# rgcgithub/regenie

Measured on AMD Instinct MI355X. Metric: Step-1 SNPs x samples x phenos / sec, higher is better.
Workload: dtype fp4 (exact integer Gram) + i8 (exact fixed-point digit planes of the fp64 operands: G~X / G~Y, many-row predictions) + f64 (solves, level 1); 1 GPU; BASELINE configs[1]: synthetic PLINK bed 50000 samples x 100000 SNPs (100000 per GPU), 1 QT pheno, bsize 1000, 22 chromosomes, 5-fold CV, 5x5 ridge grid; `value` is the HBM-resident figure (packed genotypes generated on the device, timed region = level 0 + level 1 + LOCO rows); the complete run from files on disk is `end_to_end_from_files`; samples=50000, snps=100000, phenos=1, bsize=1000, blocks=109, parallelism=blocks sharded x1, all-gather of W, level-1 Gram tiles / ridge systems shared x1

## Files before the change

include/rg_step1.h:

```cpp
#ifndef RG_STEP1_H
#define RG_STEP1_H

#include <stdint.h>

#ifdef __cplusplus
extern "C" {
#endif

typedef struct rg_ctx rg_ctx;

#define RG_OK 0
#define RG_ERR_ARG (-1)
#define RG_ERR_HIP (-2)
#define RG_ERR_LOW_VARIANCE (-3)
#define RG_ERR_NOT_SPD (-4)
#define RG_ERR_STATE (-5)

#define RG_MEM_HOST 0
#define RG_MEM_DEVICE 1

typedef struct rg_problem {
  int64_t n_samples;
  int64_t n_file;
  int32_t n_pheno;
// ... 74 lines not shown
typedef struct rg_bt_options {
  int32_t niter_max_ridge;
  int32_t niter_max_line_search_ridge;
  int32_t niter_max_line_search;
  int32_t family;
  double l1_ridge_tol;
  double tol;
  double* beta_out;
  double* fold_cumsum_out;
} rg_bt_options;
int rg_l1_bt(rg_ctx* ctx, int32_t n_ridge_l1, const double* tau, const double* yraw,
             const double* offset, const rg_bt_options* opt, int32_t nchr,
             const int32_t* cols_per_chr, double* cumsum_out, int32_t* converged_out,
             int32_t* best_out, double* pred_out);

typedef struct rg_cox_options {
  int32_t niter_max;
  int32_t niter_max_line_search;
  int32_t niter_max_ridge;
  int32_t niter_max_line_search_ridge;
  double numtol_cox;
  double l1_ridge_tol;
  const double* tau;
} rg_cox_options;
int rg_l1_cox(rg_ctx* ctx, int32_t pheno, int32_t n_ridge_l1, const double* time, const double* event, const double* offset,
              const rg_cox_options* opt, int32_t nchr, const int32_t* cols_per_chr, double* tau_out, double* deviance_out,
              int32_t* converged_out, int32_t* best_out, double* pred_out);

typedef struct rg_timing {
  double ms_prep, ms_xy, ms_gram, ms_assemble, ms_chol, ms_solve, ms_pred, ms_l1_gram, ms_l1_chol,
      ms_l1_pred;
  int64_t n_gram_launches, n_chol_launches;
  double ms_wgram;
  double ms_irls_solve;
  double ms_irls_stream;
  int64_t n_wgram;
  int64_t n_irls_rounds;
  int64_t wgram_positions;
  int64_t n_wgram_approx_rounds;
  int64_t n_irls_passes;
} rg_timing;
int rg_enable_timing(rg_ctx* ctx, int on);
int rg_get_timing(rg_ctx* ctx, rg_timing* out);

int rg_k_gram_i8(void* stream, const uint8_t* A, int64_t lda, int a_miss, const uint8_t* B,
                 int64_t ldb, int b_miss, int32_t m, int32_t n, int64_t k_bytes, int32_t* C,
                 int64_t ldc);
int rg_k_gram_fp4(void* stream, const uint8_t* A4, int64_t lda, const uint8_t* B4, int64_t ldb,
                  int32_t m, int32_t n, int64_t k_bytes, int32_t* C, int64_t ldc);
int rg_k_chol_solve(void* stream, double* mats, int64_t mat_stride, int32_t batch, int32_t n_pad,
                    int32_t rhs_pad, int32_t nrhs ,
                    double* dinv_ws ,
                    int32_t* info );
int rg_k_dgemm_nt(void* stream, const double* A, int64_t lda, const double* B, int64_t ldb,
                  int32_t m, int32_t n, int64_t k, double* C, int64_t ldc);

int rg_k_xy_i8(void* stream, const uint8_t* pk, int64_t pk_ld, int64_t pk_blk_stride, int32_t nblk, int32_t n128,
               const int32_t* bs, const int32_t* nmiss, int32_t nseg, const int64_t* fold_len, const double* V, int64_t Np,
               int32_t Cv, int32_t route, int32_t* S32, int64_t s32_elems, double* part, int64_t part_elems,
               int32_t* nchunk_out);
int rg_k_wgram(void* stream, const double* W, int64_t Np, int32_t L, int32_t P, int32_t p, const double* wv, int32_t nchain,
               int32_t nseg, const int64_t* fold_len, const int32_t* slot_chain, int32_t nslot, int32_t excl_own, int32_t fmt,
               double* out, int32_t* nslice_out);

int rg_k_mfma_peak(int kind, int iters, double* tera_ops_out);

#ifdef __cplusplus
}
#endif
#endif
```

regenie_amd/csrc/chol_p128.h:

```cpp
#pragma once
#include "chol_common.h"

#ifndef RG_HOST_EMU
#define C128_LDS_ADDR(p) ((uint32_t)(uintptr_t)(__attribute__((address_space(3))) uint8_t*)(p))
#define C128_STAGE_SYNC() asm volatile("s_waitcnt vmcnt(0) lgkmcnt(0)\n\ts_barrier" ::: "memory")
#define c128_glds16 glds16
#define C128_RFL(x) __builtin_amdgcn_readfirstlane(x)
#define C128_LDS_BARRIER() asm volatile("s_waitcnt lgkmcnt(0)\n\ts_barrier" ::: "memory")
#define C128_LAUNDER(x) asm volatile("" : "+v"(x))
#define C128_STAGE_SYNC_ACC(acc)                                                                                                        \
  asm volatile("s_waitcnt vmcnt(0) lgkmcnt(0)\n\ts_barrier"                                                                            \
               : "+v"(acc[0][0]), "+v"(acc[0][1]), "+v"(acc[1][0]), "+v"(acc[1][1]), "+v"(acc[2][0]), "+v"(acc[2][1]), "+v"(acc[3][0]), \
                 "+v"(acc[3][1]), "+v"(acc[4][0]), "+v"(acc[4][1]), "+v"(acc[5][0]), "+v"(acc[5][1]), "+v"(acc[6][0]), "+v"(acc[6][1]), \
                 "+v"(acc[7][0]), "+v"(acc[7][1])                                                                                       \
               :                                                                                                                        \
               : "memory")
#define C128_STAGE_SYNC_ACCD(acc)                                                                                                       \
  asm volatile("s_waitcnt vmcnt(0) lgkmcnt(0)\n\ts_barrier"                                                                            \
               : "+v"(acc[0][0]), "+v"(acc[0][1]), "+v"(acc[1][0]), "+v"(acc[1][1]), "+v"(acc[2][0]), "+v"(acc[2][1]), "+v"(acc[3][0]), \
                 "+v"(acc[3][1]), "+v"(acc[4][1]), "+v"(acc[5][1]), "+v"(acc[6][1]), "+v"(acc[7][1])                                   \
               :                                                                                                                        \
               : "memory")
#else
#define C128_LAUNDER(x) ((void)0)
#define C128_LDS_BARRIER() __syncthreads()
#define C128_STAGE_SYNC_ACC(acc) C128_STAGE_SYNC()
#define C128_STAGE_SYNC_ACCD(acc) C128_STAGE_SYNC()
#endif

#define C128_UNIT 16384
#define C128_NBUF 4
#define C128_DIST 3
#ifndef RG_HOST_EMU
template <int N>
__device__ __forceinline__ void c128_wait_upto(int n) {
  if (N > 0 && n >= N) { asm volatile("s_waitcnt vmcnt(%0)" ::"n"(4 * N) : "memory"); return; }
  if (N > 0) c128_wait_upto<(N > 0 ? N - 1 : 0)>(n);
  else asm volatile("s_waitcnt vmcnt(0)" ::: "memory");
}
#define C128_UNIT_SYNC(later)                                          \
  do {                                                                 \
    c128_wait_upto<C128_DIST - 1>(later);                              \
    asm volatile("s_waitcnt lgkmcnt(0)\n\ts_barrier" ::: "memory");    \
  } while (0)
#else
#define C128_UNIT_SYNC(later) __syncthreads()
#endif
#define C128_STAGE 32768
#define C128_LDS (2 * C128_STAGE + 4096)

struct C128Args {
  double* mats; int64_t mat_stride; int n64;
  double* linv;
  double* dinv;
  int32_t* info;
  int j, Tp, batch, R, nplain;
  int flags;
  unsigned long long* dbg;
  FormSrc fs;
};
#ifndef RG_HOST_EMU
#define C128_T(k)                                                                        \
  do {                                                                                   \
    if (a.dbg && threadIdx.x == 0) {                                                     \
      const unsigned long long t_ = __builtin_amdgcn_s_memrealtime();                    \
      tl[k] += t_ - t_prev;                                                              \
      t_prev = t_;                                                                       \
    }                                                                                    \
  } while (0)
#define C128_TFLUSH()                                                                    \
  do {                                                                                   \
    if (a.dbg && threadIdx.x == 0)                                                       \
      for (int k_ = 1; k_ < 16; ++k_)                                                    \
        if (tl[k_]) atomicAdd(&a.dbg[k_], tl[k_]);                                       \
  } while (0)
#define C128_T0() (a.dbg ? __builtin_amdgcn_s_memrealtime() : 0ull)
#else
#define C128_T(k) ((void)0)
#define C128_TFLUSH() ((void)0)
#define C128_T0() 0ull
#endif

__device__ __forceinline__ bool c128_factor64(double (&s)[CT][CT + 2], double (&dv)[CT], unsigned long long* dbg = nullptr) {
#ifndef RG_HOST_EMU
#define C128_FT(k) do { if (dbg && threadIdx.x == 0) { const unsigned long long t_ = __builtin_amdgcn_s_memrealtime(); dbg[k] += t_ - tf; tf = t_; } } while (0)
  unsigned long long tf = dbg ? __builtin_amdgcn_s_memrealtime() : 0ull;
#else
#define C128_FT(k) ((void)0)
#endif
  const int tid = threadIdx.x;
  const int lane = tid & 63, wave = tid >> 6;
  const int li = lane & 15, lq = lane >> 4;
  auto inv_diag = [&](int o, int r, int c) -> double {
    return (c < r) ? s[o + c][o + r] : ((c == r) ? dv[o + r] : 0.0);
  };
  bool bad = false;
  for (int sb = 0; sb < 4; ++sb) {
    const int o = sb * 16;
    const int nb = 3 - sb;
    if (tid < 16) {
      double a[16], rdv[16];
#pragma unroll
      for (int c = 0; c < 16; ++c) a[c] = s[o + tid][o + c];
#pragma unroll
      for (int c = 0; c < 16; ++c) {
        const double p0 = bcast_lane(a[c], c);
        const bool ok = p0 > 0.0;
        bad |= !ok;
        const double piv = ok ? p0 : 1.0;
        double r0 = __builtin_amdgcn_rsq(piv);
        r0 = r0 * fma(-0.5 * piv * r0, r0, 1.5);
        r0 = r0 * fma(-0.5 * piv * r0, r0, 1.5);
        double d = piv * r0;
        d = fma(0.5 * r0, fma(-d, d, piv), d);
        const double rd = fma(r0, fma(-d, r0, 1.0), r0);
        rdv[c] = rd;
        a[c] = tid == c ? d : a[c] * rd;
#pragma unroll
        for (int c2 = c + 1; c2 < 16; ++c2) a[c2] = fma(-a[c], bcast_lane(a[c], c2), a[c2]);
      }
#pragma unroll
      for (int c = 0; c < 16; ++c)
        if (c <= tid) s[o + tid][o + c] = a[c];
      double v[16];
#pragma unroll
      for (int r = 0; r < 16; ++r) v[r] = (r == tid) ? 1.0 : 0.0;
#pragma unroll
      for (int j = 0; j < 16; ++j) {
        v[j] *= rdv[j];
#pragma unroll
        for (int r = j + 1; r < 16; ++r) v[r] = fma(-bcast_lane(a[j], r), v[j], v[r]);
      }
      dv[o + tid] = v[tid];
#pragma unroll
      for (int r = 0; r < 16; ++r)
        if (r > tid) s[o + tid][o + r] = v[r];
    }
    C128_FT(11);
    C128_LDS_BARRIER();
    C128_FT(14);
    if (wave < nb) {
      const int rb = o + 16 + 16 * wave;
      v4d acc = (v4d){0, 0, 0, 0};
#pragma unroll
      for (int st = 0; st < 4; ++st)
        acc = __builtin_amdgcn_mfma_f64_16x16x4f64(s[rb + li][o + 4 * lq + st], inv_diag(o, li, 4 * lq + st), acc, 0, 0, 0);
#pragma unroll
      for (int r = 0; r < 4; ++r) s[rb + lq + 4 * r][o + li] = acc[r];
    }
    C128_LDS_BARRIER();
    {
      const int nblk2 = nb * (nb + 1) / 2;
      for (int idx = wave; idx < nblk2; idx += 4) {
        int bi = 0, rem = idx;
        while (rem > bi) { rem -= bi + 1; ++bi; }
        const int bj = rem;
        const int ri = o + 16 + 16 * bi, rj = o + 16 + 16 * bj;
        v4d acc = (v4d){0, 0, 0, 0};
#pragma unroll
        for (int st = 0; st < 4; ++st)
          acc = __builtin_amdgcn_mfma_f64_16x16x4f64(s[ri + li][o + 4 * lq + st], s[rj + li][o + 4 * lq + st], acc, 0, 0, 0);
#pragma unroll
        for (int r = 0; r < 4; ++r)
          if (bi != bj || li <= lq + 4 * r) s[ri + lq + 4 * r][rj + li] -= acc[r];
      }
    }
    C128_LDS_BARRIER();
    C128_FT(12);
  }
  C128_FT(12);
  for (int dist = 1; dist < 4; ++dist) {
    const int j = wave, ib = wave + dist;
    if (ib < 4) {
      v4d m1 = (v4d){0, 0, 0, 0};
      for (int kb = j; kb < ib; ++kb) {
#pragma unroll
        for (int st = 0; st < 4; ++st) {
          const int kk = 4 * lq + st;
          const double bval = (kb == j) ? inv_diag(16 * j, kk, li) : s[16 * j + li][16 * kb + kk];
          m1 = __builtin_amdgcn_mfma_f64_16x16x4f64(s[16 * ib + li][16 * kb + kk], bval, m1, 0, 0, 0);
        }
      }
      v4d acc = (v4d){0, 0, 0, 0};
#pragma unroll
      for (int st = 0; st < 4; ++st)
        acc = __builtin_amdgcn_mfma_f64_16x16x4f64(inv_diag(16 * ib, li, lq + 4 * st), m1[st], acc, 0, 0, 0);
#pragma unroll
      for (int r = 0; r < 4; ++r) s[16 * j + li][16 * ib + lq + 4 * r] = -acc[r];
    }
// ... 300 lines not shown
          const uint8_t* cur = smem + (u & (C128_NBUF - 1)) * C128_UNIT;
#pragma unroll
          for (int m = 0; m < 2; ++m) {
            if (m == 0 && rb > 3) continue;
            const int rbk = m == 0 ? wave : 7 - wave;
            if (rb > rbk) continue;
            const int gi = 128 * jd + 16 * rbk + i;
            const int lim = gi < nrhs ? nb - 128 * jd - q : -1;
            const int de = 16 * rbk + i - q;
            const double dadd = gi < nb ? sh : (gi < nrhs ? RG_EMBED_DIAG : 1.0), dmul = gi < nb ? 1.0 : 0.0;
#pragma unroll
            for (int r = 0; r < 4; ++r) {
              double x = c128_cols16_at(cur, 16 * rbk + i, r, i, q);
              x = (16 * rb + 4 * r < lim) ? x : 0.0;
              if (src == 0) {
                x = (16 * rb + 4 * r == de) ? fma(x, dmul, dadd) : x;
                acc[rb][m][r] -= x;
              } else {
                acc[rb][m][r] += x;
              }
            }
          }
        }
        ++u;
      }
    }
    if (MODE >= 1) {
#pragma unroll 1
      while (kc < nK) k_unit();
    }
    C128_STAGE_SYNC();
  }
  C128_T(4);
  int tid = threadIdx.x;
  C128_LAUNDER(tid);
  const int lane = tid & 63;
  const int i = lane & 15, q = lane >> 4;
  double (&sA)[CT][CT + 2] = *reinterpret_cast<double (*)[CT][CT + 2]>(smem);
  double (&sB)[CT][CT + 2] = *reinterpret_cast<double (*)[CT][CT + 2]>(smem + CT * (CT + 2) * 8);
  double (&dv)[CT] = *reinterpret_cast<double (*)[CT]>(smem + 2 * CT * (CT + 2) * 8);
  const int li = i, lq = q;
  bool bad = false;
  double* Dg = M + (int64_t)(128 * jd) * n64 + 128 * jd;
  double* Lv = a.linv + ((int64_t)b * a.Tp + jd) * (128 * 128);
  double* Iv = a.dinv + ((int64_t)b * (n64 / CT) + 2 * jd) * (CT * CT);
  auto inv_at = [&](int r, int c) -> double {
    return sA[c][r] * (c < r ? 1.0 : 0.0) + dv[r] * (c == r ? 1.0 : 0.0);
  };
  auto save_tile = [&](int o, int t) {
    for (int e = tid; e < CT * CT; e += 256) {
      const int r = e >> 6, c = e & 63;
      if (c <= r) Dg[(int64_t)(o + r) * n64 + o + c] = sA[r][c];
      const double lv = (c < r) ? sA[c][r] : (c == r ? dv[r] : 0.0);
      Lv[(o + r) * 128 + o + c] = lv;
      Iv[(int64_t)t * CT * CT + e] = lv;
    }
  };
#pragma unroll
  for (int n = 0; n < 4; ++n)
#pragma unroll
    for (int r = 0; r < 4; ++r) {
      const int rr = 16 * wave + i, cc = 16 * n + q + 4 * r;
      sA[rr][cc] = (cc <= rr) ? -acc[n][0][r] : 0.0;
    }
  C128_LDS_BARRIER();
  C128_T(6);
  if (!(a.flags & 8)) bad |= c128_factor64(sA, dv, a.dbg ? tl : nullptr);
  C128_T(7);
  const int lrb = 3 - wave;
  {
    v4d out[4];
#pragma unroll
    for (int cb = 0; cb < 4; ++cb) {
      out[cb] = (v4d){0, 0, 0, 0};
#pragma unroll
      for (int n = 0; n < 4; ++n) {
        if (n > cb) continue;
#pragma unroll
        for (int r = 0; r < 4; ++r)
          out[cb] = __builtin_amdgcn_mfma_f64_16x16x4f64(-acc[n][1][r], inv_at(16 * cb + li, 16 * n + lq + 4 * r), out[cb], 0, 0, 0);
      }
    }
#pragma unroll
    for (int cb = 0; cb < 4; ++cb)
#pragma unroll
      for (int r = 0; r < 4; ++r) {
        sB[16 * lrb + lq + 4 * r][16 * cb + li] = out[cb][r];
        Dg[(int64_t)(64 + 16 * lrb + lq + 4 * r) * n64 + 16 * cb + li] = out[cb][r];
      }
  }
  C128_LDS_BARRIER();
  v4d m1[4];
  {
#pragma unroll
    for (int cb = 0; cb < 4; ++cb) m1[cb] = (v4d){0, 0, 0, 0};
#pragma unroll 4
    for (int ks = 0; ks < 16; ++ks) {
      const int k = 4 * ks + lq;
      const double av = sB[16 * lrb + li][k];
#pragma unroll
      for (int nn = 0; nn < 4; ++nn) {
        if (nn <= lrb) acc[4 + nn][1] = __builtin_amdgcn_mfma_f64_16x16x4f64(sB[16 * nn + li][k], av, acc[4 + nn][1], 0, 0, 0);
        const int c = 16 * nn + li;
        const double bv = sA[c][k] * (c < k ? 1.0 : 0.0) + dv[k] * (c == k ? 1.0 : 0.0);
        m1[nn] = __builtin_amdgcn_mfma_f64_16x16x4f64(av, bv, m1[nn], 0, 0, 0);
      }
    }
  }
  C128_LDS_BARRIER();
  save_tile(0, 0);
  C128_LDS_BARRIER();
#pragma unroll
  for (int cb = 0; cb < 4; ++cb)
#pragma unroll
    for (int r = 0; r < 4; ++r) sB[16 * lrb + lq + 4 * r][16 * cb + li] = m1[cb][r];
#pragma unroll
  for (int nn = 0; nn < 4; ++nn)
#pragma unroll
    for (int r = 0; r < 4; ++r) {
      const int rr = 16 * lrb + i, cc = 16 * nn + q + 4 * r;
      sA[rr][cc] = (cc <= rr) ? -acc[4 + nn][1][r] : 0.0;
    }
  C128_LDS_BARRIER();
  C128_T(8);
  if (!(a.flags & 8)) bad |= c128_factor64(sA, dv, a.dbg ? tl : nullptr);
  C128_T(9);
  {
    v4d o[4];
#pragma unroll
    for (int cb = 0; cb < 4; ++cb) o[cb] = (v4d){0, 0, 0, 0};
#pragma unroll 4
    for (int ks = 0; ks < 16; ++ks) {
      const int k = 4 * ks + lq;
      const int rr = 16 * wave + li;
      const double av = sA[k][rr] * (k < rr ? 1.0 : 0.0) + dv[rr] * (k == rr ? 1.0 : 0.0);
#pragma unroll
      for (int cb = 0; cb < 4; ++cb) o[cb] = __builtin_amdgcn_mfma_f64_16x16x4f64(av, sB[k][16 * cb + li], o[cb], 0, 0, 0);
    }
#pragma unroll
    for (int cb = 0; cb < 4; ++cb)
#pragma unroll
      for (int r = 0; r < 4; ++r) Lv[(64 + 16 * wave + lq + 4 * r) * 128 + 16 * cb + li] = -o[cb][r];
  }
  save_tile(64, 1);
  C128_T(10);
  C128_TFLUSH();
  if (a.dbg && threadIdx.x == 0) { atomicAdd(&a.dbg[18], t_prev - t_start); atomicAdd(&a.dbg[21 + j], t_prev - t_start); atomicMin(&a.dbg[33 + j], t_start); atomicMax(&a.dbg[45 + j], t_prev); atomicMax(&a.dbg[64 + tl[15]], C128_T0()); }
  if (bad && !a.flags) atomicMax(a.info, 1);
}

static void c128_launch_factor(hipStream_t st, double* mats, int64_t mat_stride, int batch, int n64, double* dinv, double* linv,
                               int32_t* info, const FormSrc& first, int R, int64_t& nl) {
  C128Args a;
  a.mats = mats; a.mat_stride = mat_stride; a.n64 = n64; a.linv = linv; a.dinv = dinv; a.info = info;
  static const int flags = getenv("RG_C128_FLAGS") ? atoi(getenv("RG_C128_FLAGS")) : 0;
  if (flags & 1) R = 1;
  a.flags = flags;
  a.Tp = n64 / 128; a.batch = batch; a.R = R; a.fs = first;
  static const bool dbg = getenv("RG_C128_DBG") && atoi(getenv("RG_C128_DBG")) != 0;
  a.dbg = nullptr;
  if (dbg && hipMalloc(&a.dbg, (64 + 2048) * sizeof(unsigned long long)) == hipSuccess) {
    (void)hipMemsetAsync(a.dbg, 0, (64 + 2048) * sizeof(unsigned long long), st);
    (void)hipMemsetAsync(a.dbg + 32, 0xFF, 12 * sizeof(unsigned long long), st);
  }
  for (int j = -1; j <= a.Tp - 2; ++j) {
    a.j = j;
    a.nplain = j < 0 ? 0 : std::max(0, a.Tp - j - 2);
    const unsigned grid = xcd_affine_grid(1, batch, R) + (a.nplain ? xcd_affine_grid(a.nplain, batch, R) : 0u);
    if (j < 0) hipLaunchKernelGGL(k_c128_panel<0>, dim3(grid), dim3(256), 0, st, a);
    else if (j == 0) hipLaunchKernelGGL(k_c128_panel<1>, dim3(grid), dim3(256), 0, st, a);
    else hipLaunchKernelGGL(k_c128_panel<2>, dim3(grid), dim3(256), 0, st, a);
    ++nl;
  }
  if (a.dbg) {
    unsigned long long h[64];
    (void)hipStreamSynchronize(st);
    (void)hipMemcpy(h, a.dbg, sizeof(h), hipMemcpyDeviceToHost);
    (void)hipFree(a.dbg);
    static const char* nm[11] = {"", "X1", "K1", "T1", "X2", "K2", "->sA", "factor11", "L21/M1/D22/save", "factor22", "I21/save"};
    fprintf(stderr, "c128 phases (batch %d, n64 %d): plain items %llu, successor items %llu; workgroup-us:", batch, n64, h[16], h[17]);
    for (int k = 1; k <= 10; ++k) fprintf(stderr, " %s %.0f", nm[k], h[k] / 100.0);
    fprintf(stderr, " | prologue %.0f, workgroup lifetimes %.0f; per launch j = -1 ..:", h[19] / 100.0, h[18] / 100.0);
    for (int k = 0; k < a.Tp && k < 11; ++k) fprintf(stderr, " %.0f", h[20 + k] / 100.0);
    fprintf(stderr, " | inside the tile factorizations: 16x16 steps %.0f, barrier after them %.0f, rows below + trailing update %.0f, inverse blocks %.0f", h[11] / 100.0, h[14] / 100.0, h[12] / 100.0, h[13] / 100.0);
    fprintf(stderr, " | per launch span us (workgroups in flight):");
    for (int k = 0; k < a.Tp && k < 11; ++k) {
      const double span = (double)(h[44 + k] - h[32 + k]) / 100.0;
      fprintf(stderr, " %.0f (%.0f)", span, span > 0 ? h[20 + k] / 100.0 / span : 0.0);
    }
    fprintf(stderr, "; first start to last end of the factorization %.0f us; a CU's latest workgroup end to the next start on it: %.2f us on average over %llu starts\n",
            (double)(h[44 + a.Tp - 1] - h[32]) / 100.0, h[57] ? (double)h[56] / 100.0 / (double)h[57] : 0.0, h[57]);
  }
}
```

regenie_amd/csrc/rg_api.hip:

```cpp
#include <algorithm>
#include <cstdlib>
#include <cstring>
#include <chrono>
#include "rg_internal.h"

namespace {

template <class T>
int dev_alloc(rg_ctx* ctx, T** p, size_t n) {
  if (*p) { hipFree(*p); *p = nullptr; }
  if (n == 0) n = 1;
  RG_HIP(hipMalloc((void**)p, n * sizeof(T)));
  return RG_OK;
}
template <class T>
int dev_upload(rg_ctx* ctx, T** p, const std::vector<T>& v) {
  int rc = dev_alloc(ctx, p, v.size());
  if (rc) return rc;
  if (!v.empty()) RG_HIP(hipMemcpy(*p, v.data(), v.size() * sizeof(T), hipMemcpyHostToDevice));
  return RG_OK;
}

void free_all(rg_ctx* c) {
  void* ptrs[] = {c->d_cidx, c->d_act, c->d_V, c->d_maskp, c->d_Q, c->d_XtY, c->d_lambda, c->d_neff,
// ... 777 lines not shown
    if (chrom_ids[k] < 1 || chrom_ids[k] > nchrom) { ctx->err = "rg_set_loco_output: chromosome id out of range"; return RG_ERR_ARG; }
  ctx->loco_nchrom = nchrom;
  ctx->loco_chrom.assign(chrom_ids, chrom_ids + n_ids);
  return RG_OK;
}

int rg_set_l1_view(rg_ctx* ctx, const void* w_dev, int32_t pheno_begin, int32_t pheno_count) {
  if (!ctx || !ctx->have_problem) return RG_ERR_STATE;
  if (pheno_begin < 0 || pheno_count < 1 || pheno_begin + pheno_count > ctx->P) { ctx->err = "rg_set_l1_view: phenotype range out of bounds"; return RG_ERR_ARG; }
  ctx->v_W = (const double*)w_dev; ctx->v_p0 = pheno_begin; ctx->v_np = pheno_count;
  return RG_OK;
}

int rg_set_collective(rg_ctx* ctx, int32_t world, int32_t rank, rg_allreduce_fn fn, void* user) {
  if (!ctx) return RG_ERR_ARG;
  if (world < 1 || rank < 0 || rank >= world || (world > 1 && !fn)) { ctx->err = "rg_set_collective: bad arguments"; return RG_ERR_ARG; }
  ctx->coll_world = world; ctx->coll_rank = rank; ctx->coll_allreduce = fn; ctx->coll_user = user;
  return RG_OK;
}

int rg_enable_timing(rg_ctx* ctx, int on) {
  if (!ctx) return RG_ERR_ARG;
  ctx->timing = on != 0;
  memset(&ctx->tm, 0, sizeof(ctx->tm));
  return RG_OK;
}
int rg_get_timing(rg_ctx* ctx, rg_timing* out) {
  if (!ctx || !out) return RG_ERR_ARG;
  *out = ctx->tm;
  return RG_OK;
}

int rg_k_gram_i8(void* stream, const uint8_t* A, int64_t lda, int a_miss, const uint8_t* B,
                 int64_t ldb, int b_miss, int32_t m, int32_t n, int64_t k_bytes, int32_t* C, int64_t ldc) {
  if (!A || !B || !C || m < 1 || n < 1 || k_bytes < 16 || (k_bytes & 15) || (lda & 15) || (ldb & 15)) return RG_ERR_ARG;
  rg_launch_gram_generic((hipStream_t)stream, A, lda, a_miss, B, ldb, b_miss, m, n, k_bytes, C, ldc);
  return hipGetLastError() == hipSuccess ? RG_OK : RG_ERR_HIP;
}

int rg_k_gram_fp4(void* stream, const uint8_t* A, int64_t lda, const uint8_t* B, int64_t ldb, int32_t m,
                  int32_t n, int64_t k_bytes, int32_t* C, int64_t ldc) {
  if (!A || !B || !C || m < 1 || n < 1 || k_bytes < 128 || (k_bytes & 127) || (lda & 15) || (ldb & 15)) return RG_ERR_ARG;
  rg_launch_gram_fp4_generic((hipStream_t)stream, A, lda, B, ldb, m, n, k_bytes, C, ldc);
  return hipGetLastError() == hipSuccess ? RG_OK : RG_ERR_HIP;
}

int rg_k_chol_solve(void* stream, double* mats, int64_t mat_stride, int32_t batch, int32_t n_pad,
                    int32_t rhs_pad, int32_t nrhs, double* dinv_ws, int32_t* info) {
  if (!mats || !dinv_ws || !info || batch < 1 || n_pad < 64 || (n_pad & 63) || (rhs_pad & 63) || nrhs > rhs_pad) return RG_ERR_ARG;
  rg_launch_chol_solve((hipStream_t)stream, mats, mat_stride, batch, n_pad, rhs_pad, nrhs, dinv_ws, info, nullptr, -1);
  return hipGetLastError() == hipSuccess ? RG_OK : RG_ERR_HIP;
}

int rg_k_dgemm_nt(void* stream, const double* A, int64_t lda, const double* B, int64_t ldb, int32_t m,
                  int32_t n, int64_t k, double* C, int64_t ldc) {
  if (!A || !B || !C || (m & 63) || (n & 63) || (k & 63) || m < 64 || n < 64 || k < 64) return RG_ERR_ARG;
  rg_launch_dgemm_nt((hipStream_t)stream, A, lda, B, ldb, m, n, k, C, ldc);
  return hipGetLastError() == hipSuccess ? RG_OK : RG_ERR_HIP;
}

int rg_k_xy_i8(void* stream, const uint8_t* pk, int64_t pk_ld, int64_t pk_blk_stride, int32_t nblk, int32_t n128, const int32_t* bs,
               const int32_t* nmiss, int32_t nseg, const int64_t* fold_len, const double* V, int64_t Np, int32_t Cv, int32_t route,
               int32_t* S32, int64_t s32_elems, double* part, int64_t part_elems, int32_t* nchunk_out) {
  if (!pk || !bs || !nmiss || !fold_len || !V || nblk < 1 || n128 < 128 || (n128 % 128) || nseg < 1 || nseg > RG_MAX_SEG ||
      Cv < 1 || (route != 0 && route != 1)) return RG_ERR_ARG;
  for (int f = 0; f < nseg; ++f) if (fold_len[f] < 1) return RG_ERR_ARG;
  const SegLayout seg = rg_seg_of_lengths(fold_len, nseg);
  if (Np != seg.pos_start[nseg - 1] + seg.plen[nseg - 1] || (pk_ld & 15) || pk_ld * 4 < Np ||
      (nblk > 1 && ((pk_blk_stride & 15) || pk_blk_stride < (int64_t)n128 * pk_ld))) return RG_ERR_ARG;
  for (int b = 0; b < nblk; ++b) if (bs[b] < 1 || bs[b] > n128 || nmiss[b] < 0) return RG_ERR_ARG;
  std::vector<int64_t> cpos, clen;
  for (int f = 0; f < nseg; ++f)
    for (int64_t o = 0; o < seg.plen[f]; o += 4096) { cpos.push_back(seg.pos_start[f] + o); clen.push_back(std::min<int64_t>(4096, seg.plen[f] - o)); }
  const int nchunk = route == 0 ? nseg : (int)cpos.size();
  if (nchunk_out) *nchunk_out = nchunk;
  if (!part) return RG_OK;
  if (part_elems < (int64_t)nblk * nchunk * n128 * 2 * Cv) return RG_ERR_ARG;
  if (route == 0 && (!S32 || s32_elems < (int64_t)nblk * 2 * nseg * n128 * 128)) return RG_ERR_ARG;
  hipStream_t st = (hipStream_t)stream;
  int32_t *d_bs = nullptr, *d_nmiss = nullptr;
  int8_t* d_vd = nullptr;
  double* d_vsc = nullptr;
  int64_t *d_cpos = nullptr, *d_clen = nullptr;
  bool ok = hipMalloc(&d_bs, sizeof(int32_t) * nblk) == hipSuccess && hipMalloc(&d_nmiss, sizeof(int32_t) * nblk) == hipSuccess &&
            hipMemcpyAsync(d_bs, bs, sizeof(int32_t) * nblk, hipMemcpyHostToDevice, st) == hipSuccess &&
            hipMemcpyAsync(d_nmiss, nmiss, sizeof(int32_t) * nblk, hipMemcpyHostToDevice, st) == hipSuccess;
  if (ok && route == 0) {
    ok = hipMalloc(&d_vd, (size_t)Cv * 8 * Np) == hipSuccess && hipMalloc(&d_vsc, sizeof(double) * Cv) == hipSuccess;
    if (ok) {
      rg_launch_v_split(st, V, Np, Cv, d_vd, d_vsc);
      rg_launch_xy_i8(st, pk, pk_ld, pk_blk_stride, d_bs, d_nmiss, nblk, n128, seg, d_vd, d_vsc, Np, Cv, S32, part);
    }
  } else if (ok) {
    ok = hipMalloc(&d_cpos, sizeof(int64_t) * nchunk) == hipSuccess && hipMalloc(&d_clen, sizeof(int64_t) * nchunk) == hipSuccess &&
         hipMemcpyAsync(d_cpos, cpos.data(), sizeof(int64_t) * nchunk, hipMemcpyHostToDevice, st) == hipSuccess &&
         hipMemcpyAsync(d_clen, clen.data(), sizeof(int64_t) * nchunk, hipMemcpyHostToDevice, st) == hipSuccess;
    if (ok) rg_launch_geno_xy(st, pk, pk_ld, pk_blk_stride, d_bs, d_nmiss, nblk, n128, V, Np, Cv, d_cpos, d_clen, nchunk, part);
  }
  if (ok) ok = hipGetLastError() == hipSuccess;
  if (hipStreamSynchronize(st) != hipSuccess) ok = false;
  for (void* q : {(void*)d_bs, (void*)d_nmiss, (void*)d_vd, (void*)d_vsc, (void*)d_cpos, (void*)d_clen})
    if (q) hipFree(q);
  return ok ? RG_OK : RG_ERR_HIP;
}

}
// ... 1 lines not shown
```

regenie_amd/engine.py:

```python
from __future__ import annotations

import ctypes as C
import os
from typing import List, Optional, Sequence

import numpy as np

_LIB = None
RG_MEM_HOST, RG_MEM_DEVICE = 0, 1


class RgProblem(C.Structure):
    _fields_ = [
        ("n_samples", C.c_int64), ("n_file", C.c_int64), ("n_pheno", C.c_int32), ("n_cov", C.c_int32),
        ("cv_folds", C.c_int32), ("n_ridge_l0", C.c_int32), ("ref_first", C.c_int32),
        ("reserved0", C.c_int32), ("n_analyzed", C.c_int64), ("cv_sizes", C.c_void_p),
        ("lambda_", C.c_void_p), ("X", C.c_void_p), ("Y", C.c_void_p), ("mask", C.c_void_p),
        ("ind_in_analysis", C.c_void_p), ("ind_ignore", C.c_void_p), ("neff", C.c_void_p),
        ("n_blocks_total", C.c_int32), ("max_block_size", C.c_int32),
    ]


class RgBtOptions(C.Structure):
    _fields_ = [("niter_max_ridge", C.c_int32), ("niter_max_line_search_ridge", C.c_int32),
                ("niter_max_line_search", C.c_int32), ("family", C.c_int32),
                ("l1_ridge_tol", C.c_double), ("tol", C.c_double), ("beta_out", C.c_void_p), ("fold_cumsum_out", C.c_void_p)]


class RgCoxOptions(C.Structure):
    _fields_ = [("niter_max", C.c_int32), ("niter_max_line_search", C.c_int32), ("niter_max_ridge", C.c_int32),
                ("niter_max_line_search_ridge", C.c_int32), ("numtol_cox", C.c_double), ("l1_ridge_tol", C.c_double),
                ("tau", C.c_void_p)]


class RgTiming(C.Structure):
    _fields_ = [(n, C.c_double) for n in ("ms_prep", "ms_xy", "ms_gram", "ms_assemble", "ms_chol",
                                          "ms_solve", "ms_pred", "ms_l1_gram", "ms_l1_chol",
                                          "ms_l1_pred")] + \
               [("n_gram_launches", C.c_int64), ("n_chol_launches", C.c_int64)] + \
               [("ms_wgram", C.c_double), ("ms_irls_solve", C.c_double), ("ms_irls_stream", C.c_double),
                ("n_wgram", C.c_int64), ("n_irls_rounds", C.c_int64), ("wgram_positions", C.c_int64), ("n_wgram_approx_rounds", C.c_int64), ("n_irls_passes", C.c_int64)]

    def as_dict(self):
        return {n: getattr(self, n) for n, _ in self._fields_}


EXPORTS = ["rg_create", "rg_destroy", "rg_last_error", "rg_set_problem", "rg_set_l0_workspace", "rg_w_rows", "rg_w_bytes",
           "rg_set_w_buffer", "rg_set_block_range", "rg_w_device_ptr", "rg_l0_blocks", "rg_l0_blocks_f64", "rg_sync", "rg_l0_get_w",
           "rg_l0_set_w", "rg_l1_qt", "rg_l1_qt_loocv", "rg_l1_bt", "rg_l1_cox", "rg_set_collective", "rg_set_l1_view", "rg_set_loco_output", "rg_enable_timing", "rg_get_timing", "rg_k_gram_i8", "rg_k_gram_fp4",
           "rg_k_chol_solve", "rg_k_dgemm_nt", "rg_k_xy_i8", "rg_k_wgram", "rg_k_mfma_peak",
           "rg_group_create", "rg_group_destroy", "rg_l0_finish", "rg_group_prepare", "rg_group_abort", "rg_l0_batch_blocks", "rg_host_alloc", "rg_host_free", "rg_host_register", "rg_host_unregister",
           "rg_ingest_fence", "rg_stage_alloc", "rg_stage_copy", "rg_stage_free", "rg_stage_fits",
           "rg_pgen_open", "rg_pgen_close", "rg_pgen_last_error", "rg_pgen_info", "rg_pgen_read_bed_rows",
           "rg_pgen_read_hardcalls", "rg_pgen_set_threads", "rg_pgen_read_dosages", "rg_pgen_read_dosage_rows",
           "rg_bgen_open", "rg_bgen_close", "rg_bgen_last_error", "rg_bgen_info", "rg_bgen_sample_id", "rg_bgen_variant",
           "rg_bgen_set_threads", "rg_bgen_read_dosages", "rg_bgen_read_dosages_info", "rg_bgen_block_bytes", "rg_bgen_read_blocks",
           "rg_bgen_compressed_bytes", "rg_bgen_read_compressed", "rg_bgen_dev_create", "rg_bgen_dev_destroy", "rg_bgen_dev_last_error",
           "rg_bgen_dev_set_samples", "rg_bgen_dev_decode", "rg_bgen_dev_fetch",
           "rg_s2_create", "rg_s2_destroy", "rg_s2_last_error", "rg_s2_set_null", "rg_s2_qt_block", "rg_s2_qt_block_packed", "rg_s2_qt_block_int", "rg_s2_set_sparse_rule", "rg_s2_set_columns", "rg_s2_contract_packed", "rg_s2_contract_int", "rg_s2_bt_set_null", "rg_s2_bt_score_packed", "rg_s2_bt_score_int", "rg_s2_bt_correct",
           "rg_s2_last_kernel_ms",
           "rg_ld_create", "rg_ld_destroy", "rg_ld_last_error", "rg_ld_set_basis", "rg_ld_force_columns", "rg_ld_append", "rg_ld_finish",
           "rg_ld_pair_sums", "rg_ld_last_kernel_ms", "rg_ld_last_tiles"]


def lib_path() -> str:
    return os.path.join(os.path.dirname(os.path.abspath(__file__)), "lib", "librg_step1_hip.so")


def load_library() -> C.CDLL:
    global _LIB
    if _LIB is not None:
        return _LIB
    path = lib_path()
    if not os.path.exists(path):
        raise RuntimeError("librg_step1_hip.so is not built (%s): run `python -m regenie_amd.build` "
                           "or __graft_entry__.build()" % path)
    lib = C.CDLL(path)
    lib.rg_create.argtypes = [C.POINTER(C.c_void_p), C.c_int, C.c_void_p]
    lib.rg_destroy.argtypes = [C.c_void_p]
    lib.rg_destroy.restype = None
    lib.rg_last_error.argtypes = [C.c_void_p]
    lib.rg_last_error.restype = C.c_char_p
    lib.rg_set_problem.argtypes = [C.c_void_p, C.POINTER(RgProblem)]
    lib.rg_w_rows.argtypes = [C.c_void_p]
    lib.rg_w_rows.restype = C.c_int64
    lib.rg_w_bytes.argtypes = [C.c_void_p]
    lib.rg_w_bytes.restype = C.c_int64
    lib.rg_set_w_buffer.argtypes = [C.c_void_p, C.c_void_p, C.c_int64]
    lib.rg_w_device_ptr.argtypes = [C.c_void_p]
    lib.rg_w_device_ptr.restype = C.c_void_p
    lib.rg_l0_blocks.argtypes = [C.c_void_p, C.c_int32, C.c_void_p, C.c_void_p, C.c_void_p, C.c_int64, C.c_int]
    lib.rg_l0_blocks_f64.argtypes = [C.c_void_p, C.c_int32, C.c_void_p, C.c_void_p, C.c_void_p, C.c_int64, C.c_int]
    lib.rg_sync.argtypes = [C.c_void_p]
    lib.rg_l0_get_w.argtypes = [C.c_void_p, C.c_int32, C.c_int32, C.c_void_p]
    lib.rg_l0_set_w.argtypes = [C.c_void_p, C.c_int32, C.c_int32, C.c_void_p]
    lib.rg_l1_qt.argtypes = [C.c_void_p, C.c_int32, C.c_void_p, C.c_int32, C.c_void_p, C.c_void_p,
                             C.c_void_p, C.c_void_p]
    lib.rg_l1_qt_loocv.argtypes = lib.rg_l1_qt.argtypes
    lib.rg_l1_bt.argtypes = [C.c_void_p, C.c_int32, C.c_void_p, C.c_void_p, C.c_void_p, C.c_void_p, C.c_int32,
                             C.c_void_p, C.c_void_p, C.c_void_p, C.c_void_p, C.c_void_p]
    lib.rg_l1_cox.argtypes = [C.c_void_p, C.c_int32, C.c_int32, C.c_void_p, C.c_void_p, C.c_void_p, C.c_void_p, C.c_int32, C.c_void_p,
                              C.c_void_p, C.c_void_p, C.c_void_p, C.c_void_p, C.c_void_p]
    lib.rg_set_collective.argtypes = [C.c_void_p, C.c_int32, C.c_int32, C.c_void_p, C.c_void_p]
    lib.rg_set_l1_view.argtypes = [C.c_void_p, C.c_void_p, C.c_int32, C.c_int32]
    lib.rg_set_loco_output.argtypes = [C.c_void_p, C.c_int32, C.c_void_p, C.c_int32]
    lib.rg_set_block_range.argtypes = [C.c_void_p, C.c_int32, C.c_int32]
    lib.rg_group_create.argtypes = [C.POINTER(C.c_void_p), C.c_int32, C.POINTER(C.c_void_p), C.c_int]
    lib.rg_group_destroy.argtypes = [C.c_void_p]
    lib.rg_group_destroy.restype = None
    lib.rg_l0_finish.argtypes = [C.c_void_p, C.c_int32, C.c_void_p, C.c_void_p]
    lib.rg_l0_batch_blocks.argtypes = [C.c_void_p]
    lib.rg_l0_batch_blocks.restype = C.c_int32
    lib.rg_host_alloc.argtypes = [C.c_int64]
    lib.rg_host_alloc.restype = C.c_void_p
    lib.rg_host_free.argtypes = [C.c_void_p]
    lib.rg_host_free.restype = None
    lib.rg_ingest_fence.argtypes = [C.c_void_p]
    lib.rg_stage_alloc.argtypes = [C.c_void_p, C.c_int64, C.c_double]
    lib.rg_stage_alloc.restype = C.c_void_p
    lib.rg_stage_copy.argtypes = [C.c_void_p, C.c_void_p, C.c_void_p, C.c_int64]
    lib.rg_stage_free.argtypes = [C.c_void_p, C.c_void_p]
    lib.rg_stage_free.restype = None
    lib.rg_stage_fits.argtypes = [C.c_void_p, C.c_int64]
    lib.rg_enable_timing.argtypes = [C.c_void_p, C.c_int]
    lib.rg_get_timing.argtypes = [C.c_void_p, C.POINTER(RgTiming)]
    lib.rg_k_gram_i8.argtypes = [C.c_void_p, C.c_void_p, C.c_int64, C.c_int, C.c_void_p, C.c_int64,
                                 C.c_int, C.c_int32, C.c_int32, C.c_int64, C.c_void_p, C.c_int64]
    lib.rg_k_gram_fp4.argtypes = [C.c_void_p, C.c_void_p, C.c_int64, C.c_void_p, C.c_int64, C.c_int32, C.c_int32,
                                  C.c_int64, C.c_void_p, C.c_int64]
    lib.rg_k_chol_solve.argtypes = [C.c_void_p, C.c_void_p, C.c_int64, C.c_int32, C.c_int32,
                                    C.c_int32, C.c_int32, C.c_void_p, C.c_void_p]
    lib.rg_k_dgemm_nt.argtypes = [C.c_void_p, C.c_void_p, C.c_int64, C.c_void_p, C.c_int64,
                                  C.c_int32, C.c_int32, C.c_int64, C.c_void_p, C.c_int64]
    lib.rg_k_xy_i8.argtypes = [C.c_void_p, C.c_void_p, C.c_int64, C.c_int64, C.c_int32, C.c_int32, C.c_void_p, C.c_void_p,
                               C.c_int32, C.c_void_p, C.c_void_p, C.c_int64, C.c_int32, C.c_int32, C.c_void_p, C.c_int64,
                               C.c_void_p, C.c_int64, C.POINTER(C.c_int32)]
    lib.rg_k_wgram.argtypes = [C.c_void_p, C.c_void_p, C.c_int64, C.c_int32, C.c_int32, C.c_int32, C.c_void_p, C.c_int32,
                               C.c_int32, C.c_void_p, C.c_void_p, C.c_int32, C.c_int32, C.c_int32, C.c_void_p, C.POINTER(C.c_int32)]
    lib.rg_k_mfma_peak.argtypes = [C.c_int, C.c_int, C.POINTER(C.c_double)]
    lib.rg_pgen_open.argtypes = [C.POINTER(C.c_void_p), C.c_char_p]
    lib.rg_pgen_close.argtypes = [C.c_void_p]
    lib.rg_pgen_close.restype = None
    lib.rg_pgen_last_error.argtypes = [C.c_void_p]
    lib.rg_pgen_last_error.restype = C.c_char_p
    lib.rg_pgen_info.argtypes = [C.c_void_p, C.POINTER(C.c_int64), C.POINTER(C.c_int64), C.POINTER(C.c_int32),
                                 C.POINTER(C.c_int32), C.POINTER(C.c_int32)]
    lib.rg_pgen_read_dosages.argtypes = [C.c_void_p, C.c_int64, C.c_void_p]
    lib.rg_pgen_read_dosage_rows.argtypes = [C.c_void_p, C.c_int64, C.c_void_p, C.c_void_p, C.c_int64]
    lib.rg_s2_create.argtypes = [C.POINTER(C.c_void_p), C.c_int, C.c_int64, C.c_int32, C.c_int32]
    lib.rg_s2_destroy.argtypes = [C.c_void_p]
    lib.rg_s2_destroy.restype = None
    lib.rg_s2_last_error.argtypes = [C.c_void_p]
    lib.rg_s2_last_error.restype = C.c_char_p
    lib.rg_s2_set_null.argtypes = [C.c_void_p, C.c_void_p, C.c_void_p, C.c_void_p, C.c_void_p]
    lib.rg_s2_qt_block.argtypes = [C.c_void_p, C.c_void_p, C.c_int64, C.c_int32, C.c_int32, C.c_double, C.c_void_p]
    lib.rg_s2_qt_block_packed.argtypes = [C.c_void_p, C.c_void_p, C.c_int64, C.c_int32, C.c_int32, C.c_int32, C.c_double, C.c_void_p]
    lib.rg_s2_qt_block_int.argtypes = [C.c_void_p, C.c_void_p, C.c_int64, C.c_int32, C.c_int32, C.c_int32, C.c_double, C.c_void_p]
    lib.rg_s2_set_sparse_rule.argtypes = [C.c_void_p, C.c_int64, C.c_double, C.c_int32]
    lib.rg_s2_set_columns.argtypes = [C.c_void_p, C.c_int32, C.c_void_p, C.c_int32]
    lib.rg_s2_contract_packed.argtypes = [C.c_void_p, C.c_void_p, C.c_int64, C.c_int32, C.c_int32, C.c_int32, C.c_void_p]
    lib.rg_s2_contract_int.argtypes = [C.c_void_p, C.c_void_p, C.c_int64, C.c_int32, C.c_int32, C.c_int32, C.c_void_p]
    lib.rg_s2_bt_set_null.argtypes = [C.c_void_p, C.c_void_p]
    lib.rg_s2_bt_score_packed.argtypes = [C.c_void_p, C.c_void_p, C.c_int64, C.c_int32, C.c_int32, C.c_int32, C.c_double, C.c_void_p]
    lib.rg_s2_bt_score_int.argtypes = [C.c_void_p, C.c_void_p, C.c_int64, C.c_int32, C.c_int32, C.c_int32, C.c_double, C.c_void_p]
    lib.rg_s2_bt_correct.argtypes = [C.c_void_p, C.c_int32, C.c_int32, C.c_void_p, C.c_void_p, C.c_void_p, C.c_int32, C.c_void_p]
    lib.rg_s2_last_kernel_ms.argtypes = [C.c_void_p]
    lib.rg_s2_last_kernel_ms.restype = C.c_double
    lib.rg_bgen_open.argtypes = [C.POINTER(C.c_void_p), C.c_char_p]
    lib.rg_bgen_close.argtypes = [C.c_void_p]
    lib.rg_bgen_close.restype = None
    lib.rg_bgen_last_error.argtypes = [C.c_void_p]
    lib.rg_bgen_last_error.restype = C.c_char_p
    lib.rg_bgen_info.argtypes = [C.c_void_p, C.POINTER(C.c_int64), C.POINTER(C.c_int64), C.POINTER(C.c_int32), C.POINTER(C.c_int32)]
    lib.rg_bgen_sample_id.argtypes = [C.c_void_p, C.c_int64, C.POINTER(C.c_char_p)]
    lib.rg_bgen_variant.argtypes = [C.c_void_p, C.c_int64, C.POINTER(C.c_char_p), C.POINTER(C.c_uint32), C.POINTER(C.c_char_p),
                                    C.POINTER(C.c_char_p), C.POINTER(C.c_char_p), C.POINTER(C.c_int64)]
    lib.rg_bgen_set_threads.argtypes = [C.c_void_p, C.c_int32]
    lib.rg_bgen_read_dosages.argtypes = [C.c_void_p, C.c_int64, C.c_void_p, C.c_int32, C.c_void_p, C.c_int64]
    lib.rg_bgen_read_dosages_info.argtypes = [C.c_void_p, C.c_int64, C.c_void_p, C.c_int32, C.c_void_p, C.c_void_p, C.c_int64]
    lib.rg_bgen_block_bytes.argtypes = [C.c_void_p, C.POINTER(C.c_int64)]
    lib.rg_bgen_read_blocks.argtypes = [C.c_void_p, C.c_int64, C.c_void_p, C.c_void_p, C.c_int64, C.c_int32]
    lib.rg_bgen_compressed_bytes.argtypes = [C.c_void_p, C.c_int64, C.c_void_p, C.POINTER(C.c_int64)]
    lib.rg_bgen_read_compressed.argtypes = [C.c_void_p, C.c_int64, C.c_void_p, C.c_void_p, C.c_int64, C.c_void_p, C.c_void_p, C.c_void_p, C.c_int32]
    lib.rg_bgen_dev_create.argtypes = [C.POINTER(C.c_void_p), C.c_int32]
# ... 289 lines not shown
```

Before: 162.5 billion SNP*sample*pheno/s.

## Block the 16x16 diagonal Cholesky factor across a full wave with f64 MFMA

Replaces the 16-lane scalar factorization and inversion of each 16x16 diagonal sub-block with a whole-wave version. It works in 4x4 steps and applies the trailing updates and the inverse accumulation with f64 16x16x4 MFMA. Lane-level LDS exchange with wave barriers replaces the lane broadcasts. The aim is to shorten the serial critical path of the panel factorization in the 128-wide Cholesky used by the ridge solves. It also skips writes of the zero upper part of Lv, adds a test entry point for solving from formed sources, and limits debug phase collection. The new path adds more wave-level LDS traffic and synchronization, and it changes rounding order.

```diff
diff --git a/include/rg_step1.h b/include/rg_step1.h
--- a/include/rg_step1.h
+++ b/include/rg_step1.h
@@ -150,6 +150,9 @@
                     int32_t rhs_pad, int32_t nrhs ,
                     double* dinv_ws ,
                     int32_t* info );
+int rg_k_chol_solve_src(void* stream, const double* S, const double* F, const double* shift, int32_t nshift,
+                        const int32_t* d_n, int32_t nouter, int32_t n_pad, int32_t embed, int32_t solve,
+                        double* mats, double* dinv_ws, int32_t* info );
 int rg_k_dgemm_nt(void* stream, const double* A, int64_t lda, const double* B, int64_t ldb,
                   int32_t m, int32_t n, int64_t k, double* C, int64_t ldc);
 
diff --git a/regenie_amd/csrc/chol_p128.h b/regenie_amd/csrc/chol_p128.h
--- a/regenie_amd/csrc/chol_p128.h
+++ b/regenie_amd/csrc/chol_p128.h
@@ -8,6 +8,7 @@
 #define C128_RFL(x) __builtin_amdgcn_readfirstlane(x)
 #define C128_LDS_BARRIER() asm volatile("s_waitcnt lgkmcnt(0)\n\ts_barrier" ::: "memory")
 #define C128_LAUNDER(x) asm volatile("" : "+v"(x))
+#define C128_WAVE_SYNC() __builtin_amdgcn_wave_barrier()
 #define C128_STAGE_SYNC_ACC(acc)                                                                                                        \
   asm volatile("s_waitcnt vmcnt(0) lgkmcnt(0)\n\ts_barrier"                                                                            \
                : "+v"(acc[0][0]), "+v"(acc[0][1]), "+v"(acc[1][0]), "+v"(acc[1][1]), "+v"(acc[2][0]), "+v"(acc[2][1]), "+v"(acc[3][0]), \
@@ -23,6 +24,7 @@
                : "memory")
 #else
 #define C128_LAUNDER(x) ((void)0)
+#define C128_WAVE_SYNC() hipcpu::bar_wait(hipcpu::g_blk.wave[threadIdx.x >> 6])
 #define C128_LDS_BARRIER() __syncthreads()
 #define C128_STAGE_SYNC_ACC(acc) C128_STAGE_SYNC()
 #define C128_STAGE_SYNC_ACCD(acc) C128_STAGE_SYNC()
@@ -98,43 +100,75 @@
   for (int sb = 0; sb < 4; ++sb) {
     const int o = sb * 16;
     const int nb = 3 - sb;
-    if (tid < 16) {
-      double a[16], rdv[16];
-#pragma unroll
-      for (int c = 0; c < 16; ++c) a[c] = s[o + tid][o + c];
-#pragma unroll
-      for (int c = 0; c < 16; ++c) {
-        const double p0 = bcast_lane(a[c], c);
-        const bool ok = p0 > 0.0;
-        bad |= !ok;
-        const double piv = ok ? p0 : 1.0;
-        double r0 = __builtin_amdgcn_rsq(piv);
-        r0 = r0 * fma(-0.5 * piv * r0, r0, 1.5);
-        r0 = r0 * fma(-0.5 * piv * r0, r0, 1.5);
-        double d = piv * r0;
-        d = fma(0.5 * r0, fma(-d, d, piv), d);
-        const double rd = fma(r0, fma(-d, r0, 1.0), r0);
-        rdv[c] = rd;
-        a[c] = tid == c ? d : a[c] * rd;
-#pragma unroll
-        for (int c2 = c + 1; c2 < 16; ++c2) a[c2] = fma(-a[c], bcast_lane(a[c], c2), a[c2]);
-      }
-#pragma unroll
-      for (int c = 0; c < 16; ++c)
-        if (c <= tid) s[o + tid][o + c] = a[c];
-      double v[16];
-#pragma unroll
-      for (int r = 0; r < 16; ++r) v[r] = (r == tid) ? 1.0 : 0.0;
-#pragma unroll
-      for (int j = 0; j < 16; ++j) {
-        v[j] *= rdv[j];
-#pragma unroll
-        for (int r = j + 1; r < 16; ++r) v[r] = fma(-bcast_lane(a[j], r), v[j], v[r]);
-      }
-      dv[o + tid] = v[tid];
-#pragma unroll
-      for (int r = 0; r < 16; ++r)
-        if (r > tid) s[o + tid][o + r] = v[r];
+    if (wave == 0) {
+      v4d c, t;
+#pragma unroll
+      for (int r = 0; r < 4; ++r) {
+        c[r] = s[o + li][o + lq + 4 * r];
+        t[r] = (lq + 4 * r == li) ? 1.0 : 0.0;
+      }
+#pragma unroll
+      for (int kb = 0; kb < 4; ++kb) {
+        const int p = o + 4 * kb;
+        if (kb > 0 && li >= 4 * kb + lq) s[o + li][p + lq] = c[kb];
+        C128_WAVE_SYNC();
+        double rv[4], g[4][4], d[4], rd[4], x[4];
+#pragma unroll
+        for (int k = 0; k < 4; ++k) rv[k] = s[o + li][p + k];
+#pragma unroll
+        for (int r = 0; r < 4; ++r)
+#pragma unroll
+          for (int k = 0; k <= r; ++k) g[r][k] = s[p + r][p + k];
+        C128_WAVE_SYNC();
+#pragma unroll
+        for (int k = 0; k < 4; ++k) {
+          const double p0 = g[k][k];
+          const bool ok = p0 > 0.0;
+          bad |= !ok;
+          const double piv = ok ? p0 : 1.0;
+          double r0 = __builtin_amdgcn_rsq(piv);
+          r0 = r0 * fma(-0.5 * piv * r0, r0, 1.5);
+          r0 = r0 * fma(-0.5 * piv * r0, r0, 1.5);
+          double dd = piv * r0;
+          dd = fma(0.5 * r0, fma(-dd, dd, piv), dd);
+          d[k] = dd;
+          rd[k] = fma(r0, fma(-dd, r0, 1.0), r0);
+#pragma unroll
+          for (int r = k + 1; r < 4; ++r) g[r][k] *= rd[k];
+#pragma unroll
+          for (int r = k + 1; r < 4; ++r)
+#pragma unroll
+            for (int k2 = k + 1; k2 <= r; ++k2) g[r][k2] = fma(-g[r][k], g[k2][k], g[r][k2]);
+        }
+#pragma unroll
+        for (int k = 0; k < 4; ++k) {
+          double v = rv[k];
+#pragma unroll
+          for (int k2 = 0; k2 < k; ++k2) v = fma(-x[k2], g[k][k2], v);
+          x[k] = (li == 4 * kb + k) ? d[k] : v * rd[k];
+        }
+        const double xs = lq == 0 ? x[0] : (lq == 1 ? x[1] : (lq == 2 ? x[2] : x[3]));
+        if (li >= 4 * kb + lq) s[o + li][p + lq] = xs;
+        if (kb < 3) c = __builtin_amdgcn_mfma_f64_16x16x4f64(-xs, xs, c, 0, 0, 0);
+        double w[4];
+#pragma unroll
+        for (int j = 0; j < 4; ++j) w[j] = (j == lq) ? 1.0 : 0.0;
+#pragma unroll
+        for (int j = 0; j < 4; ++j) {
+          w[j] *= rd[j];
+#pragma unroll
+          for (int r = j + 1; r < 4; ++r) w[r] = fma(-g[r][j], w[j], w[r]);
+        }
+        const int lr = li & 3;
+        double ws = lr == 0 ? w[0] : (lr == 1 ? w[1] : (lr == 2 ? w[2] : w[3]));
+        ws = (li >> 2) == kb ? ws : 0.0;
+        const v4d xr = __builtin_amdgcn_mfma_f64_16x16x4f64(ws, t[kb], (v4d){0, 0, 0, 0}, 0, 0, 0);
+        const double iv = xr[kb];
+        const int ir = 4 * kb + lq;
+        if (ir == li) dv[o + li] = iv;
+        if (ir > li) s[o + li][o + ir] = iv;
+        if (kb < 3) t = __builtin_amdgcn_mfma_f64_16x16x4f64(-xs, iv, t, 0, 0, 0);
+      }
     }
     C128_FT(11);
     C128_LDS_BARRIER();
@@ -541,7 +575,7 @@
       const int r = e >> 6, c = e & 63;
       if (c <= r) Dg[(int64_t)(o + r) * n64 + o + c] = sA[r][c];
       const double lv = (c < r) ? sA[c][r] : (c == r ? dv[r] : 0.0);
-      Lv[(o + r) * 128 + o + c] = lv;
+      if (c < ((r >> 4) + 1) * 16) Lv[(o + r) * 128 + o + c] = lv;
       Iv[(int64_t)t * CT * CT + e] = lv;
     }
   };
@@ -648,7 +682,8 @@
   a.Tp = n64 / 128; a.batch = batch; a.R = R; a.fs = first;
   static const bool dbg = getenv("RG_C128_DBG") && atoi(getenv("RG_C128_DBG")) != 0;
   a.dbg = nullptr;
-  if (dbg && hipMalloc(&a.dbg, (64 + 2048) * sizeof(unsigned long long)) == hipSuccess) {
+  if (dbg && a.Tp > 12) fprintf(stderr, "c128 phases: not collected for n64 %d (more than 12 panels)\n", n64);
+  if (dbg && a.Tp <= 12 && hipMalloc(&a.dbg, (64 + 2048) * sizeof(unsigned long long)) == hipSuccess) {
     (void)hipMemsetAsync(a.dbg, 0, (64 + 2048) * sizeof(unsigned long long), st);
     (void)hipMemsetAsync(a.dbg + 32, 0xFF, 12 * sizeof(unsigned long long), st);
   }
diff --git a/regenie_amd/csrc/rg_api.hip b/regenie_amd/csrc/rg_api.hip
--- a/regenie_amd/csrc/rg_api.hip
+++ b/regenie_amd/csrc/rg_api.hip
@@ -853,6 +853,16 @@
   return hipGetLastError() == hipSuccess ? RG_OK : RG_ERR_HIP;
 }
 
+int rg_k_chol_solve_src(void* stream, const double* S, const double* F, const double* shift, int32_t nshift, const int32_t* d_n,
+                        int32_t nouter, int32_t n_pad, int32_t embed, int32_t solve, double* mats, double* dinv_ws, int32_t* info) {
+  if (!S || !shift || !d_n || !mats || !dinv_ws || !info || nshift < 1 || nouter < 1 || n_pad < 128 || (n_pad & 127) || embed < 0 ||
+      (solve && embed < 1)) return RG_ERR_ARG;
+  const int64_t msz = (int64_t)n_pad * n_pad;
+  rg_launch_chol_solve_formed_x((hipStream_t)stream, S, msz, F, msz, 1, shift, nshift, d_n, n_pad, nouter, mats, msz, n_pad, 0,
+                                solve ? embed : 0, dinv_ws, info, nullptr, F ? 1 : 0, nullptr, 0, 0, 1, 0, -1, 0, embed);
+  return hipGetLastError() == hipSuccess ? RG_OK : RG_ERR_HIP;
+}
+
 int rg_k_dgemm_nt(void* stream, const double* A, int64_t lda, const double* B, int64_t ldb, int32_t m,
                   int32_t n, int64_t k, double* C, int64_t ldc) {
   if (!A || !B || !C || (m & 63) || (n & 63) || (k & 63) || m < 64 || n < 64 || k < 64) return RG_ERR_ARG;
diff --git a/regenie_amd/engine.py b/regenie_amd/engine.py
--- a/regenie_amd/engine.py
+++ b/regenie_amd/engine.py
@@ -48,7 +48,7 @@
 EXPORTS = ["rg_create", "rg_destroy", "rg_last_error", "rg_set_problem", "rg_set_l0_workspace", "rg_w_rows", "rg_w_bytes",
            "rg_set_w_buffer", "rg_set_block_range", "rg_w_device_ptr", "rg_l0_blocks", "rg_l0_blocks_f64", "rg_sync", "rg_l0_get_w",
            "rg_l0_set_w", "rg_l1_qt", "rg_l1_qt_loocv", "rg_l1_bt", "rg_l1_cox", "rg_set_collective", "rg_set_l1_view", "rg_set_loco_output", "rg_enable_timing", "rg_get_timing", "rg_k_gram_i8", "rg_k_gram_fp4",
-           "rg_k_chol_solve", "rg_k_dgemm_nt", "rg_k_xy_i8", "rg_k_wgram", "rg_k_mfma_peak",
+           "rg_k_chol_solve", "rg_k_chol_solve_src", "rg_k_dgemm_nt", "rg_k_xy_i8", "rg_k_wgram", "rg_k_mfma_peak",
            "rg_group_create", "rg_group_destroy", "rg_l0_finish", "rg_group_prepare", "rg_group_abort", "rg_l0_batch_blocks", "rg_host_alloc", "rg_host_free", "rg_host_register", "rg_host_unregister",
            "rg_ingest_fence", "rg_stage_alloc", "rg_stage_copy", "rg_stage_free", "rg_stage_fits",
            "rg_pgen_open", "rg_pgen_close", "rg_pgen_last_error", "rg_pgen_info", "rg_pgen_read_bed_rows",
@@ -130,6 +130,8 @@
                                   C.c_int64, C.c_void_p, C.c_int64]
     lib.rg_k_chol_solve.argtypes = [C.c_void_p, C.c_void_p, C.c_int64, C.c_int32, C.c_int32,
                                     C.c_int32, C.c_int32, C.c_void_p, C.c_void_p]
+    lib.rg_k_chol_solve_src.argtypes = [C.c_void_p, C.c_void_p, C.c_void_p, C.c_void_p, C.c_int32, C.c_void_p, C.c_int32, C.c_int32,
+                                        C.c_int32, C.c_int32, C.c_void_p, C.c_void_p, C.c_void_p]
     lib.rg_k_dgemm_nt.argtypes = [C.c_void_p, C.c_void_p, C.c_int64, C.c_void_p, C.c_int64,
                                   C.c_int32, C.c_int32, C.c_int64, C.c_void_p, C.c_int64]
     lib.rg_k_xy_i8.argtypes = [C.c_void_p, C.c_void_p, C.c_int64, C.c_int64, C.c_int32, C.c_int32, C.c_void_p, C.c_void_p,
```

Result: faster. 165.0 billion SNP*sample*pheno/s (median of 6 runs) (+1.5%).
